# WarranWeng/EBFI-BE

Measured on AMD Instinct MI355X. Metric: interpolated frames/sec (train fwd+bwd) at B=8 256x256, higher is better.
Workload: dtype bf16x3 fwd (f16 KernelConv) / f16 bwd; 1 GPU; EVFIAutoEx (config/train_ours.yml defaults, 5.69 M params) train step: fwd + Lap/census loss + bwd + flat grad all-reduce + Adam; B=8 per GPU, 256x256 frames, TB=16 event bins, Poisson(0.35) event counts; global_batch=8, parallelism=dp1, world_size=1, launch=hipGraph replay of fwd+loss+bwd+grad packing; all-reduce and Adam eager, graph_capture_failed=False, fp16_steps_skipped=0

## Files before the change

ebfi-be_amd/csrc/conv2d.hip:

```cpp
#include <type_traits>

#include "common.hpp"
#include "c16.hpp"

using namespace ebfi;

namespace {

typedef float f32x16 __attribute__((ext_vector_type(16)));

enum { ACT_NONE = 0, ACT_LEAKY = 1, ACT_SIGMOID = 2 };

struct ConvGeom {
    int B, Cin, H, W, Cout, Ho, Wo, pad;
    int groups = 1;
    int store = 0;
};

struct EpiExtra {
    const float *addend;
    const float *mask_y;
    int mask_act;
    float mask_slope;
    _Float16 *out16 = nullptr;
// ... 3781 lines not shown
    }
    {
        ProfScope ps("conv_wgrad_f16_tr/img_batch", st, flops, bytes);
        if (int rc_ = ensure_dynamic_lds(reinterpret_cast<const void *>(&conv_wgrad_f16_tr_batch), TR_LDS + KB_LDS_BYTES)) return rc_;
        hipLaunchKernelGGL(conv_wgrad_f16_tr_batch, dim3((unsigned)(8 * 2 * n * per_xcd)), dim3(512), TR_LDS + KB_LDS_BYTES, st, bt, g0,
                           (int)tiles, per_xcd, n);
        if (int rc = check_launch("conv_wgrad_f16_tr_batch")) return rc;
    }
    {
        ProfScope ps("conv_wgrad_reduce_f32", st);
        hipLaunchKernelGGL(conv_wgrad_reduce_batch, dim3((unsigned)ceil_div(n_total_max, 64), (unsigned)n), dim3(256), 0, st, rb, 8 * per_xcd);
    }
    return check_launch("conv_wgrad_reduce_batch");
}

extern "C" int ebfi_f16_scales_finish(void *slots, int n, void *flag, void *stream) {
    if (!slots || !flag || n < 0) return fail(EBFI_ERR_ARG, "f16_scales_finish: bad argument");
    if (n == 0) return EBFI_OK;
    hipStream_t st = static_cast<hipStream_t>(stream);
    ProfScope ps("f16_scales_finish", st);
    hipLaunchKernelGGL(f16_scales_finish_kernel, dim3((unsigned)ceil_div(n, 256)), dim3(256), 0, st, static_cast<float *>(slots), n,
                       static_cast<int *>(flag));
    return check_launch("f16_scales_finish");
}

extern "C" int ebfi_pack_table_f16(const float *src, const int32_t *table, int64_t n, void *out, const int32_t *block_slot,
                                   void *slots, void *stream) {
    if (!src || !table || !out || !block_slot || !slots) return fail(EBFI_ERR_ARG, "pack_table_f16: null argument");
    if (n <= 0) return EBFI_OK;
    hipStream_t st = static_cast<hipStream_t>(stream);
// ... 39 lines not shown
```

ebfi-be_amd/csrc/conv2d_f16.inc.hpp:

```cpp


constexpr int NTF16 = 512;
template <bool EXTRA, bool IN16 = false, bool INP16 = false, bool FAC = false, bool ST = false>
__global__ __launch_bounds__(NTF16) void conv_fwd_f16_ws(const float *__restrict__ x, const _Float16 *__restrict__ wp,
                                                         const float *__restrict__ bias, float *__restrict__ out, ConvGeom g, int K16,
                                                         int act, float slope, EpiExtra epi, int tiles_total, ScaleSlot in_slot,
                                                         const float *__restrict__ w_slot, FacEpi fac) {
    static_assert(!FAC || (!EXTRA && !INP16), "the FAC epilogue comes without epilogue extras (input: fp32 planes or a c16 image)");
    constexpr int KS = 3, KK = 9, MT = 2, RW = 2;
    constexpr int IH = TYB - 1 + KS, IW = TX - 1 + KS, PS = IH * IW, COS = 32 * MT;
    constexpr int NCW = TYB / RW, PT = 256;
    constexpr int WPIECES = KK * COS * 2, NWB = (WPIECES + PT - 1) / PT;
    constexpr int INB = PS * 32, WB = KK * COS * 32, BUFB = INB + WB;
    static_assert(NCW == 4 && NTF16 == 64 * NCW + PT, "wave roles");
    extern __shared__ __attribute__((aligned(16))) char smd[];
    const int tid = threadIdx.x, lane = tid & 63, wave = tid >> 6;
    const int tiles_x = (g.Wo + TX - 1) / TX, tiles_y = (g.Ho + TYB - 1) / TYB;
    const int co_base = blockIdx.y * COS;
    const int grp = co_base / (g.Cout / g.groups);
    const int HW = g.H * g.W;
    constexpr unsigned ES = INP16 ? 2u : 4u;
    const unsigned plane_bytes = (unsigned)HW * ES, x_bytes = (unsigned)g.Cin * plane_bytes;
    const int nchunks = K16 / CKB;
    const int G = gridDim.x;
// ... 1175 lines not shown
    const int unit = pu % nunits, s_local = pu / nunits;
    WgradItem it = bt.item[0];
#pragma unroll
    for (int k = 1; k < WGRAD_BATCH_MAX; ++k)
        if (unit == k) it = bt.item[k];
    ConvGeom g = g0;
    g.Cin = it.Cin; g.Cout = it.Cout; g.groups = it.groups;
    const int t0 = (int)((int64_t)total_tiles * xcd / 8), t1 = (int)((int64_t)total_tiles * (xcd + 1) / 8);
    const bool two_co = g.Cout > 64;
    const int64_t wsz = (int64_t)g.Cout * g.Cin * 9;
    wgrad_tr_body<ACT_NONE, true, false>(static_cast<const float *>(it.x16), static_cast<const float *>(it.g16), nullptr, nullptr,
                                         it.slab + (int64_t)(xcd * per_xcd + s_local) * (wsz + g.Cout), g, 0.f, t0 + s_local, per_xcd, t1,
                                         false, it.need_bias, ScaleSlot{it.x_slot}, ScaleSlot{it.g_slot}, two_co ? which : 0,
                                         two_co ? 0 : which);
}
```

ebfi-be_amd/csrc/fuse.hip:

```cpp
#include "common.hpp"
#include "c16.hpp"

using namespace ebfi;

namespace {

typedef float f4 __attribute__((ext_vector_type(4)));

__global__ __launch_bounds__(256) void src_fwd_kernel(const float *__restrict__ a0, const float *__restrict__ s0,
                                                      const float *__restrict__ a1, const float *__restrict__ s1,
                                                      const float *__restrict__ x, float *__restrict__ out, int C, int64_t HW4,
                                                      int64_t total4, int64_t a_bs4) {
    const int64_t i = (int64_t)blockIdx.x * 256 + threadIdx.x;
    if (i >= total4) return;
    const int64_t bc = i / HW4, r = i - bc * HW4;
    const int64_t b = bc / C, c = bc - b * C;
    const f4 zero = {0.f, 0.f, 0.f, 0.f};
    const f4 xv = x ? reinterpret_cast<const f4 *>(x)[i] : zero;
    const int64_t ia = b * a_bs4 + c * HW4 + r;
    const f4 v0 = reinterpret_cast<const f4 *>(a0)[ia], v1 = reinterpret_cast<const f4 *>(a1)[ia];
    const float k0 = s0[bc], k1 = s1 ? s1[bc] : 1.f;
    f4 *o = reinterpret_cast<f4 *>(out);
    o[(b * 2 * C + c) * HW4 + r] = v0 * k0 + xv;
    o[(b * 2 * C + C + c) * HW4 + r] = v1 * k1 + xv;
// ... 53 lines not shown
    }
}

__global__ void gather_sum_kernel(const float *__restrict__ src, const int *__restrict__ idx, float *__restrict__ out,
                                  int64_t n_out, int R) {
    const int64_t i = (int64_t)blockIdx.x * blockDim.x + threadIdx.x;
    if (i >= n_out) return;
    float acc = 0.f;
    for (int r = 0; r < R; ++r) {
        const int j = idx[i * R + r];
        if (j >= 0) acc += src[j];
    }
    out[i] = acc;
}

__global__ __launch_bounds__(256) void prodmean_fwd_kernel(const float *__restrict__ a, const float *__restrict__ b,
                                                           float *__restrict__ out, int64_t HW4) {
    __shared__ float red[4];
    const f4 *pa = reinterpret_cast<const f4 *>(a) + (int64_t)blockIdx.x * HW4;
    const f4 *pb = reinterpret_cast<const f4 *>(b) + (int64_t)blockIdx.x * HW4;
    float d = 0.f;
    for (int64_t i = threadIdx.x; i < HW4; i += 256) {
        const f4 u = pa[i], v = pb[i];
        d += (u.x * v.x + u.y * v.y) + (u.z * v.z + u.w * v.w);
    }
#pragma unroll
    for (int s = 32; s >= 1; s >>= 1) d += __shfl_xor(d, s, 64);
    if ((threadIdx.x & 63) == 0) red[threadIdx.x >> 6] = d;
    __syncthreads();
    if (threadIdx.x == 0) out[blockIdx.x] = ((red[0] + red[1]) + (red[2] + red[3])) / (float)(HW4 * 4);
// ... 436 lines not shown
                           static_cast<float *>(slot), grad_x, grad_s0_part, grad_s1_part, B, C, HW / 4, W / 4, (int64_t)0, nslice,
                           mask_slope, static_cast<const float *>(a_slot));
    }
    return check_launch("scale_residual_cat_bwd");
}

extern "C" int ebfi_gather_sum(const float *src, const int32_t *idx, float *out, int64_t n_out, int R, void *stream) {
    if (!src || !idx || !out) return fail(EBFI_ERR_ARG, "gather_sum: null argument");
    if (n_out < 0 || R <= 0) return fail(EBFI_ERR_ARG, "gather_sum: bad dimensions");
    if (n_out == 0) return EBFI_OK;
    hipStream_t st = static_cast<hipStream_t>(stream);
    hipLaunchKernelGGL(gather_sum_kernel, dim3((unsigned)ceil_div(n_out, 256)), dim3(256), 0, st, src, idx, out, n_out, R);
    return check_launch("gather_sum");
}

extern "C" int ebfi_prodmean_forward(const float *a, const float *b, float *out, int64_t planes, int64_t HW, void *stream) {
    if (!a || !b || !out) return fail(EBFI_ERR_ARG, "prodmean_forward: null argument");
    if (planes < 0 || planes > 2147483647LL || HW <= 0) return fail(EBFI_ERR_ARG, "prodmean_forward: bad dimensions");
    if (HW % 4 != 0) return fail(EBFI_ERR_UNSUPPORTED, "prodmean_forward: H*W must be a multiple of 4");
    if (planes == 0) return EBFI_OK;
    hipStream_t st = static_cast<hipStream_t>(stream);
    {
        ProfScope ps("prodmean_fwd", st, 0.0, 8.0 * planes * (double)HW);
        hipLaunchKernelGGL(prodmean_fwd_kernel, dim3((unsigned)planes), dim3(256), 0, st, a, b, out, HW / 4);
    }
    return check_launch("prodmean_fwd");
}

extern "C" int ebfi_prodmean_backward(const float *a, const float *b, const float *grad_out, float *grad_a, float *grad_b,
                                      int64_t planes, int64_t HW, void *stream) {
// ... 57 lines not shown
```

ebfi-be_amd/ebfi_amd/_native.py:

```python
import ctypes
import os
import re
import subprocess
import threading

PKG_ROOT = os.path.dirname(os.path.dirname(os.path.abspath(__file__)))
REPO_ROOT = os.path.dirname(PKG_ROOT)
_DEV = os.environ.get("EBFI_DEV") == "1"


def dev_env(name, default=None):
    return os.environ.get(name, default) if _DEV else default


LIB_PATH = dev_env("EBFI_LIB_PATH") or os.path.join(PKG_ROOT, "lib", "libebfi_hip.so")
HEADER = os.path.join(REPO_ROOT, "include", "ebfi_hip.h")
BUILD_SCRIPT = os.path.join(PKG_ROOT, "csrc", "build.sh")

EBFI_F32, EBFI_F32_BF16MMA, EBFI_F32_BF16X3MMA = 0, 2, 3
EBFI_ERR_UNSUPPORTED = -3
ABI_VERSION = 14


class EbfiNativeError(RuntimeError):
# ... 32 lines not shown
    "ebfi_pack_pairs_block": (_i, []),
    "ebfi_pack_pairs_bf16": (_i, [_vp, _vp, _vp, _vp, _i64, _i64, _vp, _vp]),
    "ebfi_f16_scales_finish": (_i, [_vp, _i, _vp, _vp]),
    "ebfi_pack_table_f16": (_i, [_vp, _vp, _i64, _vp, _vp, _vp, _vp]),
    "ebfi_conv2d_packed_f16": (_i, [_vp, _vp, _sz, _vp, _vp] + [_i] * 8 + [_i, _c.c_float, _vp, _vp, _i, _c.c_float, _vp, _vp, _vp]),
    "ebfi_conv2d_backward_weight_f16g": (_i, [_vp] * 6 + [_i] * 8 + [_i, _c.c_float, _vp, _vp, _vp, _sz, _vp]),
    "ebfi_conv2d_backward_weight_f16g_ex": (_i, [_vp] * 6 + [_i] * 9 + [_i, _c.c_float, _vp, _vp, _vp, _sz, _vp]),
    "ebfi_to_c16": (_i, [_vp, _vp, _c.c_float, _vp, _vp, _i, _i, _i, _i, _vp]),
    "ebfi_to_c16_cat2": (_i, [_vp, _i, _vp, _i, _vp, _vp, _i, _i, _i, _vp]),
    "ebfi_conv2d_packed_x3_c16": (_i, [_vp, _vp, _sz, _vp, _vp] + [_i] * 8 + [_i, _c.c_float, _vp, _vp, _i, _c.c_float, _vp, _vp, _i, _vp]),
    "ebfi_conv2d_packed_f16_c16": (_i, [_vp, _i, _vp, _sz, _vp, _vp] + [_i] * 8 + [_i, _c.c_float, _vp, _vp, _i, _c.c_float,
                                        _vp, _vp, _vp, _vp, _i, _i, _vp]),
    "ebfi_conv2d_backward_weight_f16c": (_i, [_vp, _vp, _i, _vp, _vp] + [_i] * 6 + [_vp, _vp, _vp, _sz, _vp]),
    "ebfi_conv2d_backward_weight_f16c_batch_workspace": (_sz, [_i, _vp, _vp]),
    "ebfi_conv2d_backward_weight_f16c_batch": (_i, [_i] + [_vp] * 9 + [_i, _i, _i, _vp, _sz, _vp]),
    "ebfi_fac_forward_p16": (_i, [_vp, _i, _vp, _vp, _vp, _i, _i, _i, _i, _i, _vp]),
    "ebfi_fac_backward_p16": (_i, [_vp, _i, _vp, _vp, _vp, _vp, _vp, _vp, _c.c_float, _i, _i, _i, _i, _i, _vp]),
    "ebfi_scale_residual_cat_forward_c16": (_i, [_vp] * 8 + [_i, _i, _i, _i, _i64, _vp]),
    "ebfi_scale_residual_cat_backward_slices": (_i, []),
    "ebfi_scale_residual_cat_backward_c16": (_i, [_vp] * 10 + [_i, _i, _i, _i, _i64, _c.c_float, _vp]),
    "ebfi_scale_residual_cat_backward_c16a": (_i, [_vp] * 10 + [_i, _i, _i, _i, _c.c_float, _vp]),
    "ebfi_conv2d_packed_x3_rc": (_i, [_vp, _vp, _sz, _vp, _vp] + [_i] * 6 + [_c.c_float, _vp, _vp, _i, _vp, _vp, _vp, _vp, _vp]),
    "ebfi_conv2d_thin_forward": (_i, [_vp, _vp, _vp, _vp] + [_i] * 8 + [_i, _c.c_float, _vp]),
    "ebfi_kernelconv_fac_fused_x3": (_i, [_vp, _vp, _sz, _vp, _vp, _vp] + [_i] * 6 + [_c.c_float, _vp]),
    "ebfi_kernelconv_fac_fused_f16": (_i, [_vp, _i, _vp, _sz, _vp, _vp, _vp] + [_i] * 6 + [_c.c_float, _vp, _vp, _vp]),
    "ebfi_conv2d_packed_x3": (_i, [_vp, _vp, _sz, _vp, _vp] + [_i] * 8 + [_i, _c.c_float, _vp, _vp, _i, _c.c_float, _vp]),
    "ebfi_conv2d_backward_weight_x3g": (_i, [_vp] * 4 + [_i] * 8 + [_vp, _sz, _vp]),
    "ebfi_scale_residual_cat_forward_ex": (_i, [_vp] * 6 + [_i, _i, _i64, _i64, _vp]),
    "ebfi_scale_residual_cat_backward_ex": (_i, [_vp] * 10 + [_i, _i, _i64, _i64, _i64, _i, _c.c_float, _vp]),
    "ebfi_scalar_conv_forward": (_i, [_vp, _vp, _vp, _vp, _i, _i, _i, _i, _c.c_float, _vp]),
    "ebfi_scalar_conv_backward": (_i, [_vp, _vp, _vp, _vp, _vp, _vp, _vp, _i, _i, _i, _i, _c.c_float, _vp]),
    "ebfi_events_workspace": (_sz, [_i]),
    "ebfi_events_to_stack": (_i, [_vp, _vp, _vp, _vp, _i64, _i, _i, _i, _vp, _vp, _sz, _vp]),
    "ebfi_frame2lap": (_i, [_vp, _vp, _i, _i, _i, _vp]),
    "ebfi_frame2dcp": (_i, [_vp, _vp, _vp, _i, _i, _i, _i, _vp]),
    "ebfi_scale_residual_cat_forward": (_i, [_vp] * 6 + [_i, _i, _i64, _vp]),
    "ebfi_scale_residual_cat_backward": (_i, [_vp] * 10 + [_i, _i, _i64, _vp]),
    "ebfi_prodmean_forward": (_i, [_vp, _vp, _vp, _i64, _i64, _vp]),
    "ebfi_prodmean_backward": (_i, [_vp] * 5 + [_i64, _i64, _vp]),
    "ebfi_gather_sum": (_i, [_vp, _vp, _vp, _i64, _i, _vp]),
    "ebfi_se_gate_workspace": (_c.c_size_t, [_i, _i, _i64]),
    "ebfi_se_gate_forward": (_i, [_vp] * 8 + [_i, _i, _i64, _i, _c.c_float, _vp]),
    "ebfi_se_gate_backward": (_i, [_vp] * 11 + [_i, _i, _i64, _i, _c.c_float, _vp]),
    "ebfi_conv2d_packed_x3_shuffled": (_i, [_vp, _vp, _c.c_size_t, _vp, _vp] + [_i] * 6 + [_c.c_float, _i, _vp]),
    "ebfi_conv2d_packed_f16_shuffled": (_i, [_vp, _i, _vp, _c.c_size_t, _vp, _vp] + [_i] * 6 + [_c.c_float, _vp, _i, _c.c_float, _vp, _vp, _i, _vp]),
    "ebfi_se_gate_forward_ps": (_i, [_vp] * 7 + [_i, _i, _i, _i, _i, _c.c_float, _vp]),
    "ebfi_se_gate_backward_ps": (_i, [_vp] * 10 + [_i, _i, _i, _i, _i, _c.c_float, _vp]),
    "ebfi_groupnorm_workspace": (_sz, [_i, _i]),
    "ebfi_groupnorm_forward": (_i, [_vp] * 6 + [_i, _i, _i64, _i, _c.c_float, _vp, _sz, _vp]),
    "ebfi_groupnorm_backward": (_i, [_vp] * 8 + [_i, _i, _i64, _i, _vp, _sz, _vp]),
    "ebfi_census_partials": (_i64, [_i, _i, _i]),
    "ebfi_census_forward": (_i, [_vp, _vp, _vp, _i, _i, _i, _i, _vp]),
    "ebfi_census_backward": (_i, [_vp, _vp, _vp, _vp, _i, _i, _i, _i, _vp]),
    "ebfi_census_pair_forward": (_i, [_vp, _vp, _vp, _c.c_float, _c.c_float, _vp, _vp, _i, _i, _i, _i, _vp]),
    "ebfi_census_pair_backward": (_i, [_vp, _vp, _vp, _c.c_float, _c.c_float, _vp, _vp, _vp, _i, _i, _i, _i, _vp]),
# ... 177 lines not shown
```

ebfi-be_amd/ebfi_amd/conv.py:

```python
import os

import torch
import torch.nn.functional as F
from torch.autograd import Function

from . import _native as N

ACT_NONE, ACT_LEAKY, ACT_SIGMOID = 0, 1, 2

_COMPUTE = "fp32"
MODES = ("fp32", "bf16x3", "bf16")


def set_compute_dtype(mode):
    global _COMPUTE
    if mode not in MODES:
        raise ValueError("compute dtype must be one of %s" % (MODES,))
    _COMPUTE = mode


def get_compute_dtype():
    return _COMPUTE


# ... 175 lines not shown
        if Cin != site.K:
            raise RuntimeError("input has %d channels, the packed weight expects %d" % (Cin, site.K))
        geo = [B, Cin, H, W, site.M, site.ks, 1, int(pad)]
        Ho, Wo = H + 2 * pad - site.ks + 1, W + 2 * pad - site.ks + 1
        out = torch.empty((B, site.M, Ho, Wo), dtype=x.dtype, device=x.device)
        with torch.cuda.device_of(x):
            if site.kind == "id" and len(site.w_shapes) == 1 and site.groups == 1 and \
                    _thin_forward(x, params[0].contiguous(), site.bias(), out, geo, act, slope):
                rc = 0
            else:
                rc = N.lib().ebfi_conv2d_forward_bf16x3(N.ptr(x), N.ptr(None), N.ptr(site.bias()), N.ptr(out), *geo, act, slope,
                                                        site.fwd_ptr(), site.fwd_bytes, N.stream_ptr(x.device))
        N.check(rc, "ebfi_conv2d_forward_bf16x3 (packed)")
        if grad_preact:
            act, slope = ACT_NONE, 0.0
        ctx.site, ctx.cfg, ctx.geo = site, (act, slope), geo
        ctx.save_for_backward(x, out if act != ACT_NONE else None)
        return out

    @staticmethod
    def backward(ctx, gout):
        x, y = ctx.saved_tensors
        site, (act, slope), geo = ctx.site, ctx.cfg, ctx.geo
        gx, pgrads = _site_backward(site, geo, act, slope, x, y, gout, ctx.needs_input_grad[0], any(ctx.needs_input_grad[6:]))
        return (gx, None, None, None, None, None) + tuple(pgrads)


def _site_backward(site, geo, act, slope, x, y, gout, need_x, need_p, unshuffle=None):
    gout = gout.contiguous()
    lib = N.lib()
    gx, pgrads = None, [None] * (len(site.w_shapes) + len(site.b_shapes))
    from . import f16scale
    book = f16scale.active_book()
    B, Cin, H, W, M, ks, _, pad = geo
    f16 = book is not None and ks == 3 and pad == 1
    al16 = all(t is None or t.data_ptr() % 16 == 0 for t in (x, gout, y))
    f16_w = f16 and (Cin % 64 == 0 or (Cin >= 32 and W % 4 == 0 and al16))
    f16_x = f16 and W % 4 == 0 and Cin >= 48 and site.tr16_ptr() is not None
    gpre = None

    def weight_gradients(st_w):
        gw2 = torch.empty((site.M, site.K, site.ks, site.ks), dtype=x.dtype, device=x.device)
        gb2 = torch.empty(site.M, dtype=x.dtype, device=x.device) if site.has_bias else None
        need = int(lib.ebfi_conv2d_backward_weight_workspace(*geo, N.EBFI_F32))
        ws = torch.empty(max(need, 4), dtype=torch.uint8, device=x.device)
        gpre16 = need_x and act != ACT_NONE and f16_w and f16_x and al16 and W % 4 == 0 and M % 16 == 0 and site.groups == 1
        gp = None
        if need_x and act != ACT_NONE:
            if gpre16:
                from . import c16
                gp = c16.empty(B, M, H, W, x.device)
            else:
                gp = torch.empty_like(gout)
        if f16_w:
            rc = lib.ebfi_conv2d_backward_weight_f16g_ex(N.ptr(x), N.ptr(gout), N.ptr(y), N.ptr(gw2), N.ptr(gb2), N.ptr(gp),
                                                         1 if gpre16 else 0, B, Cin, H, W, M, ks, pad, 1, act, slope,
                                                         book.operand((site.key, "x"), x), book.operand((site.key, "g"), gout),
                                                         N.ptr(ws), need, st_w)
        else:
            rc = lib.ebfi_conv2d_backward_weight_ex(N.ptr(x), N.ptr(gout), N.ptr(y), N.ptr(gw2), N.ptr(gb2), N.ptr(gp), *geo,
                                                    act, slope, N.ptr(ws), need, N.EBFI_F32_BF16X3MMA, st_w)
        N.check(rc, "ebfi_conv2d_backward_weight")
        return _route_site_grads(site, gw2, gb2, st_w), gp

    with torch.cuda.device_of(x):
        st = N.stream_ptr(x.device)
        if need_p:
            pgrads, gpre = weight_gradients(st)
        if need_x:
            src, sy, a = (gpre, None, ACT_NONE) if gpre is not None else (gout, y, act)
            img = gpre is not None and gpre.dtype == torch.float16
            native_unshuffle = unshuffle is not None and (img or (f16_x and a == ACT_NONE)) and site.groups == 1 and H % 2 == 0 and \
                W % 4 == 0 and Cin > 32 and unshuffle[0].is_contiguous() and unshuffle[0].data_ptr() % 16 == 0
            if native_unshuffle:
                gx = torch.empty((B, 4 * Cin, H // 2, W // 2), dtype=x.dtype, device=x.device)
                in_slot = book.ptr(book.slot((site.key, "g"))) if img else book.operand((site.key, "g"), src)
                rc = lib.ebfi_conv2d_packed_f16_shuffled(N.ptr(src), 1 if img else 0, site.tr16_ptr(), site.tr16_bytes, N.ptr(None), N.ptr(gx),
                                                         B, M, H, W, Cin, ACT_NONE, 0.0, N.ptr(unshuffle[0]), ACT_LEAKY, float(unshuffle[1]),
                                                         in_slot, site.w_slot_ptr(), 2, st)
                N.check(rc, "ebfi_conv2d_packed_f16_shuffled (data gradient through the inverse pixel shuffle)")
                return gx, pgrads
            gx = torch.empty_like(x)
# ... 28 lines not shown
        if Cin != site_a.K or site_a.M != 4 * site_b.K:
            raise RuntimeError("shuffled pair: %d -> %d channels, then %d -> %d" % (Cin, site_a.M, site_b.K, site_b.M))
        geo_a = [B, Cin, H, W, site_a.M, 3, 1, 1]
        geo_b = [B, site_b.K, 2 * H, 2 * W, site_b.M, 3, 1, 1]
        y1 = torch.empty((B, site_b.K, 2 * H, 2 * W), dtype=x.dtype, device=x.device)
        y2 = torch.empty((B, site_b.M, 2 * H, 2 * W), dtype=x.dtype, device=x.device)
        with torch.cuda.device_of(x):
            st = N.stream_ptr(x.device)
            rc = N.lib().ebfi_conv2d_packed_x3_shuffled(N.ptr(x), site_a.fwd_ptr(), site_a.fwd_bytes, N.ptr(site_a.bias()), N.ptr(y1), B, Cin,
                                                        H, W, site_a.M, ACT_LEAKY, slope_a, 1, st)
            N.check(rc, "ebfi_conv2d_packed_x3_shuffled")
            rc = N.lib().ebfi_conv2d_forward_bf16x3(N.ptr(y1), N.ptr(None), N.ptr(site_b.bias()), N.ptr(y2), *geo_b, act_b, slope_b,
                                                    site_b.fwd_ptr(), site_b.fwd_bytes, st)
            N.check(rc, "ebfi_conv2d_forward_bf16x3 (packed)")
        ctx.sites, ctx.cfg, ctx.geos, ctx.na = (site_a, site_b), (slope_a, act_b, slope_b), (geo_a, geo_b), na
        ctx.save_for_backward(x, y1, y2 if act_b != ACT_NONE else None)
        return y2

    @staticmethod
    def backward(ctx, g2):
        x, y1, y2 = ctx.saved_tensors
        (site_a, site_b), (slope_a, act_b, slope_b), (geo_a, geo_b), na = ctx.sites, ctx.cfg, ctx.geos, ctx.na
        need = ctx.needs_input_grad
        need_pa, need_pb = any(need[7:7 + na]), any(need[7 + na:])
        need_a = need[0] or need_pa
        ga, pg_b = _site_backward(site_b, geo_b, act_b, slope_b, y1, y2, g2, need_a, need_pb, unshuffle=(y1, slope_a))
        gx, pg_a = (None, [None] * na)
        if need_a:
            gx, pg_a = _site_backward(site_a, geo_a, ACT_NONE, 0.0, x, None, ga, need[0], need_pa)
        return (gx, None, None, None, None, None, None) + tuple(pg_a) + tuple(pg_b)


def shuffle_pair_usable(x, site_a, site_b):
    return (site_usable(site_a, x) and site_b is not None and site_a.ks == 3 and site_b.ks == 3 and site_a.kind == "id" and
            site_b.kind == "id" and site_a.groups == 1 and site_b.groups == 1 and site_a.M == 4 * site_b.K and site_a.M > 32 and
            x.shape[3] % 4 == 0 and x.data_ptr() % 16 == 0 and not torch.is_autocast_enabled())


def conv_shuffle_pair(x, site_a, slope_a, params_a, site_b, act_b, slope_b, params_b):
    return SiteConvShufflePair.apply(x, site_a, float(slope_a), site_b, int(act_b), float(slope_b), len(params_a), *params_a, *params_b)


def _route_site_grads(site, gw2, gb2, st):
    lib = N.lib()
# ... 38 lines not shown
```

ebfi-be_amd/ebfi_amd/engine.py:

```python
import contextlib

import torch

from . import graphstep
from .dp import FlatGradBucket, broadcast_parameters, build_flat_optimizer
from .loss import TrainLoss
from .model import EVFIAutoEx

DEFAULT_MODEL_ARGS = dict(
    FrameBasech=64, EventBasech=64, InterCH=64, TB=16, norm=None, activation="LeakyReLU",
    UseGTEx=False, FixEx=None, BlurryFashion="RGBLap", BLInch=4, UseEvents=True, LoadPretrainEX=False,
    PretrainedEXPath=None, FrozenEX=False, step=12, DualPath=True, residual=True, DetailEnabled=True,
    channels=[16, 24, 32, 64])


def synthetic_batch(B, H, W, TB=16, device="cuda", seed=123, rank=0, on_device=False):
    dev = torch.device(device)
    if on_device and dev.type == "cuda":
        g = torch.Generator(device=dev).manual_seed(seed + rank)
        rnd = lambda *shape: torch.rand(*shape, generator=g, device=dev)
        frame = rnd(B, 3, H, W)
        event = torch.poisson(torch.full((B, TB, 2, H, W), 0.35, device=dev), generator=g)
        t = rnd(B, 1)
        gtex = rnd(B, 1) * 0.4 + 0.55
# ... 27 lines not shown


def synthetic_validation_batch(B, H, W, TB=16, num_frames=4, device="cuda", seed=0):
    g = torch.Generator(device="cpu").manual_seed(int(seed))
    frame = torch.rand(B, 3, H, W, generator=g)
    event = torch.poisson(torch.full((B, TB, 2, H, W), 0.35), generator=g)
    gtex = torch.rand(B, 1, generator=g) * 0.4 + 0.55
    latent = torch.rand(B, num_frames, 3, H, W, generator=g)
    ts = (torch.arange(num_frames) / num_frames).expand(B, num_frames).contiguous()
    return tuple(v.to(device) for v in (frame, event, ts, gtex, latent))


class Engine(graphstep.GraphStepper):
    def __init__(self, model_args=None, device="cuda", precision="fp32", lr=1e-4, seed=None, train=True, graph=False,
                 accu_step=1, betas=(0.9, 0.999), backward_f16=None, forward_f16="filters", strict_graph=None,
                 perceptual=None, optimizer=None):
        if precision not in ("fp32", "bf16x3", "bf16"):
            raise ValueError("precision must be 'fp32', 'bf16x3' or 'bf16'")
        super().__init__(device, graph=graph, accu_step=accu_step, strict_graph=strict_graph)
        self.precision = precision
        if seed is not None:
            torch.manual_seed(seed)
        self.model_args = dict(DEFAULT_MODEL_ARGS, **(model_args or {}))
        self.model = EVFIAutoEx(**self.model_args).to(self.device)
        broadcast_parameters(self.model, 0)
        self.calibration_steps = 2
        self.perceptual = perceptual if train else None
        self.keep_panels, self.panel_sharp, self.last_valid_panels = False, None, None
        if train:
            self.model.train()
            self.loss = TrainLoss(self.model_args.get("DetailEnabled", True)).to(self.device)
            self.bucket = FlatGradBucket(self.model)
            self.optimizer = build_flat_optimizer(self.bucket.params, optimizer, lr, betas)
        else:
            self.model.eval()
        self.bank = None
        if backward_f16 is None:
            backward_f16 = True
        use_book = train and precision == "bf16x3" and backward_f16
        forward_f16 = forward_f16 if use_book else None
        if forward_f16 == "none":
# ... 7 lines not shown
                                             fwd16=forward_f16) if train else weightbank.build_for(self.model, inference=True)
        self.book = None
        if use_book and self.bank is not None:
            from . import f16scale
            self.book = f16scale.ScaleBook(self.device)
            self.bank.attach_scale_book(self.book)
            self.bank.pack_on_demand = True
            self.book.forward_f16 = forward_f16

    def _book(self):
        if self.book is None or self.precision != "bf16x3":
            return contextlib.nullcontext()
        return self.book.active()

    def _fwd_bwd(self, frame, event, t, gtex, target):
        with self._autocast(), self._bank(), self._book() as book:
            if book is not None and self._steps_run < self.calibration_steps:
                book.calibrated.clear()
            sharp_pre, sharp = self.model(frame, event, t, gtex)
            if self.keep_panels:
                if self.panel_sharp is None or self.panel_sharp.shape[1:] != sharp.shape[1:]:
                    self.panel_sharp = torch.empty((1,) + tuple(sharp.shape[1:]), dtype=torch.float32, device=sharp.device)
                self.panel_sharp.copy_(sharp.detach()[:1])
            loss = self.loss(sharp_pre.float(), sharp.float(), target, self.iteration, self.accu_step)
            if self.perceptual is not None:
                loss = loss + self.perceptual(sharp.float(), target) / self.accu_step
            loss.backward()
            if book is not None:
                book.finish()
        return loss.detach()

    def _begin_micro_step(self):
        if self.book is not None and self.precision == "bf16x3" and self._micro == 0:
            self.book.begin_step()

    def _guard(self):
        return self.book.guard if (self.book is not None and self.precision == "bf16x3") else None

    def _calibrating(self):
        return self.book is not None and self.precision == "bf16x3" and self._steps_run < self.calibration_steps

    def _graph_key(self):
# ... 190 lines not shown
```

include/ebfi_hip.h:

```cpp
#ifndef EBFI_HIP_H
#define EBFI_HIP_H

#include <stddef.h>
#include <stdint.h>

#ifdef __cplusplus
extern "C" {
#endif

#define EBFI_ABI_VERSION 14

typedef enum {
    EBFI_OK = 0,
    EBFI_ERR_ARG = -1,
    EBFI_ERR_LAUNCH = -2,
    EBFI_ERR_UNSUPPORTED = -3,
    EBFI_ERR_WORKSPACE = -4
} ebfi_status;

typedef enum { EBFI_F32 = 0, EBFI_F32_BF16MMA = 2, EBFI_F32_BF16X3MMA = 3 } ebfi_dtype;

int ebfi_abi_version(void);
const char *ebfi_last_error(void);

// ... 132 lines not shown
int ebfi_conv2d_packed_x3_shuffled(const void *input, const void *packed, size_t packed_bytes, const void *bias, void *output,
                                   int B, int Cin, int H, int W, int Cout, int act, float slope, int out_layout, void *stream);
int ebfi_conv2d_packed_f16_shuffled(const void *input, int input_is_c16, const void *packed16, size_t packed_bytes,
                                    const void *bias, void *output, int B, int Cin, int H, int W, int Cout, int act, float slope,
                                    const void *mask_y, int mask_act, float mask_slope, void *in_slot, const void *w_slot,
                                    int out_layout, void *stream);
int ebfi_conv2d_backward_weight_f16c(const void *input16, const void *grad16, int grad_is_planar, void *grad_weight,
                                     void *grad_bias, int B, int Cin_per_group, int H, int W, int Cout, int groups,
                                     const void *x_slot, const void *g_slot, void *workspace, size_t workspace_bytes,
                                     void *stream);
size_t ebfi_conv2d_backward_weight_f16c_batch_workspace(int n, const int *Cin_per_group, const int *Cout);
int ebfi_conv2d_backward_weight_f16c_batch(int n, const void *const *input16, const void *const *grad16, void *const *grad_weight,
                                           void *const *grad_bias, const int *Cin_per_group, const int *Cout, const int *groups,
                                           void *const *x_slot, void *const *g_slot, int B, int H, int W, void *workspace,
                                           size_t workspace_bytes, void *stream);
int ebfi_fac_forward_p16(const float *input, int input_is_unpadded, const void *filters16, const void *f_slot, float *output, int B,
                         int C, int Ho, int Wo, int K, void *stream);
int ebfi_fac_backward_p16(const float *input, int input_is_unpadded, const void *filters16, const void *f_slot,
                          const float *grad_output, float *grad_input, void *grad_kernel16, void *g_slot, float kernel_leaky_slope,
                          int B, int C, int Ho, int Wo, int K, void *stream);
int ebfi_scale_residual_cat_forward_c16(const float *a0, const float *s0, const float *a1, const float *s1, const float *x,
                                        float *out, void *out16, void *slot, int B, int C, int H, int W,
                                        int64_t a_batch_stride, void *stream);
int ebfi_scale_residual_cat_backward_slices(void);
int ebfi_scale_residual_cat_backward_c16(const float *grad_out, const float *a0, const float *s0, const float *a1,
                                         const float *s1, void *grad_a16, void *slot, float *grad_x, float *grad_s0_part,
                                         float *grad_s1_part, int B, int C, int H, int W, int64_t a_batch_stride,
                                         float mask_slope, void *stream);
int ebfi_scale_residual_cat_backward_c16a(const float *grad_out, const void *a16, const void *a_slot, const float *s0, const float *s1,
                                          void *grad_a16, void *slot, float *grad_x, float *grad_s0_part, float *grad_s1_part, int B,
// ... 27 lines not shown
                                     const float *s1, float *grad_a0, float *grad_a1, float *grad_x,
                                     float *grad_s0, float *grad_s1, int B, int C, int64_t HW, void *stream);

int ebfi_scale_residual_cat_forward_ex(const float *a0, const float *s0, const float *a1, const float *s1, const float *x,
                                       float *out, int B, int C, int64_t HW, int64_t a_batch_stride, void *stream);
int ebfi_scale_residual_cat_backward_ex(const float *grad_out, const float *a0, const float *s0, const float *a1,
                                        const float *s1, float *grad_a0, float *grad_a1, float *grad_x, float *grad_s0,
                                        float *grad_s1, int B, int C, int64_t HW, int64_t a_batch_stride,
                                        int64_t grad_a_batch_stride, int mask_leaky, float mask_slope, void *stream);

int ebfi_prodmean_forward(const float *a, const float *b, float *out, int64_t planes, int64_t HW, void *stream);
int ebfi_prodmean_backward(const float *a, const float *b, const float *grad_out, float *grad_a, float *grad_b,
                           int64_t planes, int64_t HW, void *stream);

int ebfi_gather_sum(const float *src, const int32_t *idx, float *out, int64_t n_out, int R, void *stream);

size_t ebfi_se_gate_workspace(int B, int C, int64_t N);
int ebfi_se_gate_forward(const float *x, const float *weight, const float *bias, const float *res, float *out, float *mean,
                         float *gate, float *workspace, int B, int C, int64_t N, int act, float slope, void *stream);
int ebfi_se_gate_backward(const float *grad_out, const float *out, const float *x, const float *weight, const float *gate,
                          const float *mean, float *grad_x, float *grad_res, float *grad_weight, float *grad_bias,
                          float *workspace, int B, int C, int64_t N, int act, float slope, void *stream);

int ebfi_se_gate_forward_ps(const float *x, const float *weight, const float *bias, float *out, float *mean, float *gate,
                            float *workspace, int B, int C, int h, int w, int act, float slope, void *stream);
int ebfi_se_gate_backward_ps(const float *grad_out, const float *out, const float *x, const float *weight, const float *gate,
                             const float *mean, float *grad_x, float *grad_weight, float *grad_bias, float *workspace, int B, int C,
                             int h, int w, int act, float slope, void *stream);

size_t ebfi_groupnorm_workspace(int B, int C);
// ... 148 lines not shown
```

Before: 568.7 frames/s.

## Defer conv weight gradients into a batched multi-layer wgrad and gather launch

Adds a weight-gradient queue that collects eligible 3x3 conv layers during backward and computes all their weight gradients at the end in one grouped kernel plus one grouped reduce. Per-parameter gather-sum routing is batched the same way through a multi-item gather kernel. The aim is fewer small launches and better GPU fill for small layers whose wgrad underuses the device. In exchange, activations and output gradients stay alive until the flush, which raises peak memory, and wgrad work no longer overlaps with the dgrad chain.

```diff
diff --git a/ebfi-be_amd/csrc/conv2d.hip b/ebfi-be_amd/csrc/conv2d.hip
--- a/ebfi-be_amd/csrc/conv2d.hip
+++ b/ebfi-be_amd/csrc/conv2d.hip
@@ -3819,6 +3819,121 @@
     return check_launch("conv_wgrad_reduce_batch");
 }
 
+namespace {
+struct ReduceMultiItem {
+    const float *slab;
+    float *gw, *gb;
+    int64_t n_weight, n_total;
+    int perm_cin, nslabs;
+};
+struct ReduceMulti {
+    ReduceMultiItem item[WGRAD_MULTI_MAX];
+};
+__global__ __launch_bounds__(256) void conv_wgrad_reduce_multi(ReduceMulti rb) {
+    const ReduceMultiItem &it = rb.item[blockIdx.y];
+    if ((int64_t)blockIdx.x * 64 >= it.n_total) return;
+    wgrad_reduce_body(it.slab, it.nslabs, it.n_weight, it.n_total, it.gw, it.gb, it.perm_cin, 9);
+}
+
+int64_t wgrad_multi_tiles(const ConvGeom &g) { return (int64_t)g.B * ceil_div(g.Ho, TRH) * ceil_div(g.Wo, TRW); }
+void wgrad_multi_plan(const ConvGeom *g, int n, int *nsplit) {
+    for (int k = 0; k < n; ++k) {
+        const int64_t tiles = wgrad_multi_tiles(g[k]);
+        const int s = wgrad_x3_splits(g[k], 3);
+        nsplit[k] = (int)(s > tiles ? tiles : s);
+    }
+}
+size_t wgrad_multi_slab_bytes(const ConvGeom &g, int nsplit) {
+    const size_t b = (size_t)nsplit * ((size_t)g.Cout * g.Cin * 9 + g.Cout) * sizeof(float);
+    return (b + 255) / 256 * 256;
+}
+}
+
+extern "C" size_t ebfi_conv2d_backward_weight_f16g_multi_workspace(int n, const int *B, const int *Cin, const int *H, const int *W,
+                                                                   const int *Cout) {
+    if (n < 1 || !B || !Cin || !H || !W || !Cout) return 0;
+    size_t total = 0;
+    for (int k0 = 0; k0 < n; k0 += WGRAD_MULTI_MAX) {
+        const int m = n - k0 < WGRAD_MULTI_MAX ? n - k0 : WGRAD_MULTI_MAX;
+        ConvGeom g[WGRAD_MULTI_MAX];
+        int ns[WGRAD_MULTI_MAX];
+        for (int k = 0; k < m; ++k)
+            if (B[k0 + k] < 1 || make_geom(g[k], B[k0 + k], Cin[k0 + k], H[k0 + k], W[k0 + k], Cout[k0 + k], 3, 1, 1) != EBFI_OK) return 0;
+        wgrad_multi_plan(g, m, ns);
+        for (int k = 0; k < m; ++k) total += wgrad_multi_slab_bytes(g[k], ns[k]);
+    }
+    return total;
+}
+
+extern "C" int ebfi_conv2d_backward_weight_f16g_multi(int n, const void *const *input, const void *const *grad_output,
+                                                      void *const *grad_weight, void *const *grad_bias, const int *B, const int *Cin,
+                                                      const int *H, const int *W, const int *Cout, const int *ksize, const int *stride,
+                                                      const int *pad, const int *groups, void *const *x_slot, void *const *g_slot,
+                                                      void *workspace, size_t workspace_bytes, void *stream) {
+    if (n < 1) return fail(EBFI_ERR_ARG, "conv2d_backward_weight_f16g_multi: %d layers", n);
+    if (!input || !grad_output || !grad_weight || !grad_bias || !B || !Cin || !H || !W || !Cout || !ksize || !stride || !pad || !groups ||
+        !x_slot || !g_slot)
+        return fail(EBFI_ERR_ARG, "conv2d_backward_weight_f16g_multi: null argument");
+    for (int k = 0; k < n; ++k) {
+        if (!input[k] || !grad_output[k] || !grad_weight[k]) return fail(EBFI_ERR_ARG, "conv2d_backward_weight_f16g_multi: null argument (layer %d)", k);
+        if (ksize[k] != 3 || stride[k] != 1 || pad[k] != 1 || groups[k] != 1 || B[k] < 1 || Cin[k] < 16 || W[k] % 4 != 0 ||
+            !aligned16(input[k]) || !aligned16(grad_output[k]))
+            return fail(EBFI_ERR_UNSUPPORTED, "conv2d_backward_weight_f16g_multi: layer %d (k=%d stride %d pad %d, %d groups, %d -> %d channels, "
+                                              "W=%d) is not a 3x3 same-padded stride-1 layer on quad-aligned rows with >= 16 input channels and "
+                                              "16-byte aligned operands", k, ksize[k], stride[k], pad[k], groups[k], Cin[k], Cout[k], W[k]);
+        ConvGeom g;
+        if (int rc = make_geom(g, B[k], Cin[k], H[k], W[k], Cout[k], 3, 1, 1)) return rc;
+        if (shift_wgrad_geometry(g, 3, 1).kind != 0 || thin_wgrad_geometry(g, 3, 1).kind != 0)
+            return fail(EBFI_ERR_UNSUPPORTED, "conv2d_backward_weight_f16g_multi: layer %d (%d -> %d) is a thin layer with kernels of its own", k,
+                        Cin[k], Cout[k]);
+        if (wgrad_multi_tiles(g) > 2147483647LL / 4) return fail(EBFI_ERR_ARG, "conv2d_backward_weight_f16g_multi: too many tiles (layer %d)", k);
+    }
+    const size_t need = ebfi_conv2d_backward_weight_f16g_multi_workspace(n, B, Cin, H, W, Cout);
+    if (!workspace || workspace_bytes < need)
+        return fail(EBFI_ERR_WORKSPACE, "conv2d_backward_weight_f16g_multi: workspace %zu bytes < required %zu", workspace_bytes, need);
+    hipStream_t st = static_cast<hipStream_t>(stream);
+    char *ws = static_cast<char *>(workspace);
+    for (int k0 = 0; k0 < n; k0 += WGRAD_MULTI_MAX) {
+        const int m = n - k0 < WGRAD_MULTI_MAX ? n - k0 : WGRAD_MULTI_MAX;
+        ConvGeom g[WGRAD_MULTI_MAX];
+        int ns[WGRAD_MULTI_MAX];
+        for (int k = 0; k < m; ++k) (void)make_geom(g[k], B[k0 + k], Cin[k0 + k], H[k0 + k], W[k0 + k], Cout[k0 + k], 3, 1, 1);
+        wgrad_multi_plan(g, m, ns);
+        WgradMulti mt{};
+        ReduceMulti rb{};
+        double flops = 0.0, bytes = 0.0;
+        int64_t wgs = 0, n_total_max = 0;
+        for (int k = 0; k < m; ++k) {
+            const int i = k0 + k;
+            const int64_t n_weight = (int64_t)g[k].Cout * g[k].Cin * 9, n_total = n_weight + g[k].Cout;
+            float *slab = reinterpret_cast<float *>(ws);
+            ws += wgrad_multi_slab_bytes(g[k], ns[k]);
+            mt.item[k] = WgradMultiItem{static_cast<const float *>(input[i]), static_cast<const float *>(grad_output[i]), slab,
+                                        static_cast<float *>(x_slot[i]), static_cast<float *>(g_slot[i]), g[k].B, g[k].Cin, g[k].H, g[k].W,
+                                        g[k].Cout, ns[k], (int)wgrad_multi_tiles(g[k]), grad_bias[i] != nullptr ? 1 : 0, (int)wgs, 0};
+            rb.item[k] = ReduceMultiItem{slab, static_cast<float *>(grad_weight[i]), static_cast<float *>(grad_bias[i]), n_weight, n_total,
+                                         g[k].Cin, ns[k]};
+            wgs += ceil_div((int64_t)ns[k] * ceil_div(g[k].Cout, 64) * ceil_div(g[k].Cin, 64), 8) * 8;
+            n_total_max = n_total > n_total_max ? n_total : n_total_max;
+            flops += 2.0 * g[k].B * g[k].Ho * g[k].Wo * (double)g[k].Cout * g[k].Cin * 9;
+            bytes += conv_bytes_wgrad(g[k], 9, false, false);
+        }
+        if (wgs > 2147483647LL) return fail(EBFI_ERR_ARG, "conv2d_backward_weight_f16g_multi: too many workgroups");
+        {
+            ProfScope ps("conv_wgrad_f16_tr/f32_multi", st, flops, bytes);
+            if (int rc_ = ensure_dynamic_lds(reinterpret_cast<const void *>(&conv_wgrad_f16_tr_multi), TR_LDS + KB_LDS_BYTES)) return rc_;
+            hipLaunchKernelGGL(conv_wgrad_f16_tr_multi, dim3((unsigned)wgs), dim3(512), TR_LDS + KB_LDS_BYTES, st, mt, m);
+            if (int rc = check_launch("conv_wgrad_f16_tr_multi")) return rc;
+        }
+        {
+            ProfScope ps("conv_wgrad_reduce_f32", st);
+            hipLaunchKernelGGL(conv_wgrad_reduce_multi, dim3((unsigned)ceil_div(n_total_max, 64), (unsigned)m), dim3(256), 0, st, rb);
+            if (int rc = check_launch("conv_wgrad_reduce_multi")) return rc;
+        }
+    }
+    return EBFI_OK;
+}
+
 extern "C" int ebfi_f16_scales_finish(void *slots, int n, void *flag, void *stream) {
     if (!slots || !flag || n < 0) return fail(EBFI_ERR_ARG, "f16_scales_finish: bad argument");
     if (n == 0) return EBFI_OK;
diff --git a/ebfi-be_amd/csrc/conv2d_f16.inc.hpp b/ebfi-be_amd/csrc/conv2d_f16.inc.hpp
--- a/ebfi-be_amd/csrc/conv2d_f16.inc.hpp
+++ b/ebfi-be_amd/csrc/conv2d_f16.inc.hpp
@@ -1213,3 +1213,44 @@
                                          false, it.need_bias, ScaleSlot{it.x_slot}, ScaleSlot{it.g_slot}, two_co ? which : 0,
                                          two_co ? 0 : which);
 }
+
+struct WgradMultiItem {
+    const float *x, *gout;
+    float *slab, *x_slot, *g_slot;
+    int B, Cin, H, W, Cout;
+    int nsplit, total_tiles, need_bias;
+    int wg_begin, pad_;
+};
+constexpr int WGRAD_MULTI_MAX = 16;
+struct WgradMulti {
+    WgradMultiItem item[WGRAD_MULTI_MAX];
+};
+__global__ __launch_bounds__(512) void conv_wgrad_f16_tr_multi(WgradMulti mt, int n) {
+    int k = 0;
+    for (int j = 1; j < n; ++j)
+        if ((int)blockIdx.x >= mt.item[j].wg_begin) k = j;
+    const WgradMultiItem &it = mt.item[k];
+    const int nx = it.nsplit, ny = (it.Cout + 63) / 64, nz = (it.Cin + 63) / 64;
+    const int L = (int)blockIdx.x - it.wg_begin, total = nx * ny * nz;
+    if (L >= total) return;
+    int split, co_blk, ci_blk;
+    {
+        const int T8 = total / (8 * nz) * (8 * nz);
+        int rest;
+        if (L < T8) {
+            const int xcd = L & 7, i = L >> 3;
+            ci_blk = i % nz;
+            rest = (i / nz) * 8 + xcd;
+        } else {
+            ci_blk = (L - T8) % nz;
+            rest = T8 / nz + (L - T8) / nz;
+        }
+        split = rest % nx;
+        co_blk = rest / nx;
+    }
+    ConvGeom g{it.B, it.Cin, it.H, it.W, it.Cout, it.H, it.W, 1};
+    const int64_t wsz = (int64_t)g.Cout * g.Cin * 9;
+    wgrad_tr_body<ACT_NONE, false, false>(it.x, it.gout, nullptr, nullptr, it.slab + (int64_t)split * (wsz + g.Cout), g, 0.f, split, nx,
+                                          it.total_tiles, (nx & 7) == 0, it.need_bias, ScaleSlot{it.x_slot}, ScaleSlot{it.g_slot},
+                                          co_blk, ci_blk, 0);
+}
diff --git a/ebfi-be_amd/csrc/fuse.hip b/ebfi-be_amd/csrc/fuse.hip
--- a/ebfi-be_amd/csrc/fuse.hip
+++ b/ebfi-be_amd/csrc/fuse.hip
@@ -91,6 +91,35 @@
     out[i] = acc;
 }
 
+struct GatherItem {
+    const float *src;
+    const int *idx;
+    float *out;
+    int64_t n_out;
+    int R, wg_begin;
+};
+constexpr int GATHER_MULTI_MAX = 48;
+struct GatherMulti {
+    GatherItem item[GATHER_MULTI_MAX];
+};
+__global__ __launch_bounds__(256) void gather_sum_multi_kernel(GatherMulti gm, int n) {
+    int k = 0;
+    for (int j = 1; j < n; ++j)
+        if ((int)blockIdx.x >= gm.item[j].wg_begin) k = j;
+    const GatherItem &it = gm.item[k];
+    const int64_t i = (int64_t)((int)blockIdx.x - it.wg_begin) * 256 + threadIdx.x;
+    if (i >= it.n_out) return;
+    const int R = it.R;
+    const int *__restrict__ idx = it.idx;
+    const float *__restrict__ src = it.src;
+    float acc = 0.f;
+    for (int r = 0; r < R; ++r) {
+        const int j = idx[i * R + r];
+        if (j >= 0) acc += src[j];
+    }
+    it.out[i] = acc;
+}
+
 __global__ __launch_bounds__(256) void prodmean_fwd_kernel(const float *__restrict__ a, const float *__restrict__ b,
                                                            float *__restrict__ out, int64_t HW4) {
     __shared__ float red[4];
@@ -557,6 +586,37 @@
     return check_launch("gather_sum");
 }
 
+extern "C" int ebfi_gather_sum_multi(int n, const float *const *src, const int32_t *const *idx, float *const *out, const int64_t *n_out,
+                                     const int *R, void *stream) {
+    if (n < 0 || !src || !idx || !out || !n_out || !R) return fail(EBFI_ERR_ARG, "gather_sum_multi: bad argument");
+    for (int k = 0; k < n; ++k) {
+        if (!src[k] || !idx[k] || !out[k]) return fail(EBFI_ERR_ARG, "gather_sum_multi: null argument (item %d)", k);
+        if (n_out[k] < 0 || R[k] <= 0) return fail(EBFI_ERR_ARG, "gather_sum_multi: bad dimensions (item %d)", k);
+    }
+    hipStream_t st = static_cast<hipStream_t>(stream);
+    int k = 0;
+    while (k < n) {
+        GatherMulti gm{};
+        int m = 0;
+        int64_t wgs = 0;
+        for (; k < n && m < GATHER_MULTI_MAX; ++k) {
+            if (n_out[k] == 0) continue;
+            const int64_t w = ceil_div(n_out[k], 256);
+            if (wgs + w > 2147483647LL) {
+                if (m == 0) return fail(EBFI_ERR_ARG, "gather_sum_multi: item %d is too large", k);
+                break;
+            }
+            gm.item[m++] = GatherItem{src[k], idx[k], out[k], n_out[k], R[k], (int)wgs};
+            wgs += w;
+        }
+        if (m == 0) break;
+        ProfScope ps("gather_sum", st);
+        hipLaunchKernelGGL(gather_sum_multi_kernel, dim3((unsigned)wgs), dim3(256), 0, st, gm, m);
+        if (int rc = check_launch("gather_sum_multi")) return rc;
+    }
+    return EBFI_OK;
+}
+
 extern "C" int ebfi_prodmean_forward(const float *a, const float *b, float *out, int64_t planes, int64_t HW, void *stream) {
     if (!a || !b || !out) return fail(EBFI_ERR_ARG, "prodmean_forward: null argument");
     if (planes < 0 || planes > 2147483647LL || HW <= 0) return fail(EBFI_ERR_ARG, "prodmean_forward: bad dimensions");
diff --git a/ebfi-be_amd/ebfi_amd/_native.py b/ebfi-be_amd/ebfi_amd/_native.py
--- a/ebfi-be_amd/ebfi_amd/_native.py
+++ b/ebfi-be_amd/ebfi_amd/_native.py
@@ -70,6 +70,8 @@
     "ebfi_conv2d_backward_weight_f16c": (_i, [_vp, _vp, _i, _vp, _vp] + [_i] * 6 + [_vp, _vp, _vp, _sz, _vp]),
     "ebfi_conv2d_backward_weight_f16c_batch_workspace": (_sz, [_i, _vp, _vp]),
     "ebfi_conv2d_backward_weight_f16c_batch": (_i, [_i] + [_vp] * 9 + [_i, _i, _i, _vp, _sz, _vp]),
+    "ebfi_conv2d_backward_weight_f16g_multi_workspace": (_sz, [_i] + [_vp] * 5),
+    "ebfi_conv2d_backward_weight_f16g_multi": (_i, [_i] + [_vp] * 15 + [_vp, _sz, _vp]),
     "ebfi_fac_forward_p16": (_i, [_vp, _i, _vp, _vp, _vp, _i, _i, _i, _i, _i, _vp]),
     "ebfi_fac_backward_p16": (_i, [_vp, _i, _vp, _vp, _vp, _vp, _vp, _vp, _c.c_float, _i, _i, _i, _i, _i, _vp]),
     "ebfi_scale_residual_cat_forward_c16": (_i, [_vp] * 8 + [_i, _i, _i, _i, _i64, _vp]),
@@ -95,6 +97,7 @@
     "ebfi_prodmean_forward": (_i, [_vp, _vp, _vp, _i64, _i64, _vp]),
     "ebfi_prodmean_backward": (_i, [_vp] * 5 + [_i64, _i64, _vp]),
     "ebfi_gather_sum": (_i, [_vp, _vp, _vp, _i64, _i, _vp]),
+    "ebfi_gather_sum_multi": (_i, [_i, _vp, _vp, _vp, _vp, _vp, _vp]),
     "ebfi_se_gate_workspace": (_c.c_size_t, [_i, _i, _i64]),
     "ebfi_se_gate_forward": (_i, [_vp] * 8 + [_i, _i, _i64, _i, _c.c_float, _vp]),
     "ebfi_se_gate_backward": (_i, [_vp] * 11 + [_i, _i, _i64, _i, _c.c_float, _vp]),
diff --git a/ebfi-be_amd/ebfi_amd/conv.py b/ebfi-be_amd/ebfi_amd/conv.py
--- a/ebfi-be_amd/ebfi_amd/conv.py
+++ b/ebfi-be_amd/ebfi_amd/conv.py
@@ -213,7 +213,7 @@
         N.check(rc, "ebfi_conv2d_forward_bf16x3 (packed)")
         if grad_preact:
             act, slope = ACT_NONE, 0.0
-        ctx.site, ctx.cfg, ctx.geo = site, (act, slope), geo
+        ctx.site, ctx.cfg, ctx.geo, ctx.params = site, (act, slope), geo, params
         ctx.save_for_backward(x, out if act != ACT_NONE else None)
         return out
 
@@ -221,11 +221,12 @@
     def backward(ctx, gout):
         x, y = ctx.saved_tensors
         site, (act, slope), geo = ctx.site, ctx.cfg, ctx.geo
-        gx, pgrads = _site_backward(site, geo, act, slope, x, y, gout, ctx.needs_input_grad[0], any(ctx.needs_input_grad[6:]))
+        gx, pgrads = _site_backward(site, geo, act, slope, x, y, gout, ctx.needs_input_grad[0], any(ctx.needs_input_grad[6:]),
+                                    params=(ctx.params, ctx.needs_input_grad[6:]))
         return (gx, None, None, None, None, None) + tuple(pgrads)
 
 
-def _site_backward(site, geo, act, slope, x, y, gout, need_x, need_p, unshuffle=None):
+def _site_backward(site, geo, act, slope, x, y, gout, need_x, need_p, unshuffle=None, params=None):
     gout = gout.contiguous()
     lib = N.lib()
     gx, pgrads = None, [None] * (len(site.w_shapes) + len(site.b_shapes))
@@ -237,6 +238,8 @@
     f16_w = f16 and (Cin % 64 == 0 or (Cin >= 32 and W % 4 == 0 and al16))
     f16_x = f16 and W % 4 == 0 and Cin >= 48 and site.tr16_ptr() is not None
     gpre = None
+    from . import wgradqueue
+    queue = wgradqueue.active() if params is not None and need_p and wgradqueue.deferrable(*params) else None
 
     def weight_gradients(st_w):
         gw2 = torch.empty((site.M, site.K, site.ks, site.ks), dtype=x.dtype, device=x.device)
@@ -260,11 +263,16 @@
             rc = lib.ebfi_conv2d_backward_weight_ex(N.ptr(x), N.ptr(gout), N.ptr(y), N.ptr(gw2), N.ptr(gb2), N.ptr(gp), *geo,
                                                     act, slope, N.ptr(ws), need, N.EBFI_F32_BF16X3MMA, st_w)
         N.check(rc, "ebfi_conv2d_backward_weight")
+        if queue is not None and site.kind != "id":
+            queue.add_routes(site, gw2, gb2, *params)
+            return pgrads, gp
         return _route_site_grads(site, gw2, gb2, st_w), gp
 
     with torch.cuda.device_of(x):
         st = N.stream_ptr(x.device)
-        if need_p:
+        if need_p and queue is not None and f16_w and wgradqueue.eligible(site, geo, act, x, gout):
+            queue.add_layer(site, x, gout, geo, book.operand((site.key, "x"), x), book.operand((site.key, "g"), gout), *params)
+        elif need_p:
             pgrads, gpre = weight_gradients(st)
         if need_x:
             src, sy, a = (gpre, None, ACT_NONE) if gpre is not None else (gout, y, act)
@@ -323,6 +331,7 @@
                                                     site_b.fwd_ptr(), site_b.fwd_bytes, st)
             N.check(rc, "ebfi_conv2d_forward_bf16x3 (packed)")
         ctx.sites, ctx.cfg, ctx.geos, ctx.na = (site_a, site_b), (slope_a, act_b, slope_b), (geo_a, geo_b), na
+        ctx.params = params
         ctx.save_for_backward(x, y1, y2 if act_b != ACT_NONE else None)
         return y2
 
@@ -333,10 +342,12 @@
         need = ctx.needs_input_grad
         need_pa, need_pb = any(need[7:7 + na]), any(need[7 + na:])
         need_a = need[0] or need_pa
-        ga, pg_b = _site_backward(site_b, geo_b, act_b, slope_b, y1, y2, g2, need_a, need_pb, unshuffle=(y1, slope_a))
+        ga, pg_b = _site_backward(site_b, geo_b, act_b, slope_b, y1, y2, g2, need_a, need_pb, unshuffle=(y1, slope_a),
+                                  params=(ctx.params[na:], need[7 + na:]))
         gx, pg_a = (None, [None] * na)
         if need_a:
-            gx, pg_a = _site_backward(site_a, geo_a, ACT_NONE, 0.0, x, None, ga, need[0], need_pa)
+            gx, pg_a = _site_backward(site_a, geo_a, ACT_NONE, 0.0, x, None, ga, need[0], need_pa,
+                                      params=(ctx.params[:na], need[7:7 + na]))
         return (gx, None, None, None, None, None, None) + tuple(pg_a) + tuple(pg_b)
 
 
diff --git a/ebfi-be_amd/ebfi_amd/engine.py b/ebfi-be_amd/ebfi_amd/engine.py
--- a/ebfi-be_amd/ebfi_amd/engine.py
+++ b/ebfi-be_amd/ebfi_amd/engine.py
@@ -65,7 +65,7 @@
 class Engine(graphstep.GraphStepper):
     def __init__(self, model_args=None, device="cuda", precision="fp32", lr=1e-4, seed=None, train=True, graph=False,
                  accu_step=1, betas=(0.9, 0.999), backward_f16=None, forward_f16="filters", strict_graph=None,
-                 perceptual=None, optimizer=None):
+                 perceptual=None, optimizer=None, defer_wgrad=True, defer_wgrad_cap=None):
         if precision not in ("fp32", "bf16x3", "bf16"):
             raise ValueError("precision must be 'fp32', 'bf16x3' or 'bf16'")
         super().__init__(device, graph=graph, accu_step=accu_step, strict_graph=strict_graph)
@@ -76,6 +76,7 @@
         self.model = EVFIAutoEx(**self.model_args).to(self.device)
         broadcast_parameters(self.model, 0)
         self.calibration_steps = 2
+        self.defer_wgrad, self.defer_wgrad_cap = bool(defer_wgrad), defer_wgrad_cap
         self.perceptual = perceptual if train else None
         self.keep_panels, self.panel_sharp, self.last_valid_panels = False, None, None
         if train:
@@ -113,7 +114,10 @@
         return self.book.active()
 
     def _fwd_bwd(self, frame, event, t, gtex, target):
-        with self._autocast(), self._bank(), self._book() as book:
+        from . import wgradqueue
+        cap = wgradqueue.BYTE_CAP if self.defer_wgrad_cap is None else self.defer_wgrad_cap
+        with self._autocast(), self._bank(), self._book() as book, \
+                wgradqueue.scope(self.defer_wgrad and self.book is not None, cap) as queue:
             if book is not None and self._steps_run < self.calibration_steps:
                 book.calibrated.clear()
             sharp_pre, sharp = self.model(frame, event, t, gtex)
@@ -125,6 +129,8 @@
             if self.perceptual is not None:
                 loss = loss + self.perceptual(sharp.float(), target) / self.accu_step
             loss.backward()
+            if queue is not None:
+                queue.flush()
             if book is not None:
                 book.finish()
         return loss.detach()
diff --git a/ebfi-be_amd/ebfi_amd/wgradqueue.py b/ebfi-be_amd/ebfi_amd/wgradqueue.py
--- /dev/null
+++ b/ebfi-be_amd/ebfi_amd/wgradqueue.py
@@ -0,0 +1,140 @@
+import contextlib
+import ctypes
+
+import torch
+
+from . import _native as N
+
+BYTE_CAP = 1 << 30
+
+_ACTIVE = None
+
+
+def active():
+    return _ACTIVE
+
+
+def deferrable(params, needs):
+    return all((not n) or (p.is_leaf and p.requires_grad) for p, n in zip(params, needs))
+
+
+def eligible(site, geo, act, x, gout):
+    B, Cin, H, W, M, ks, _, pad = geo
+    return (act == 0 and ks == 3 and pad == 1 and site.groups == 1 and W % 4 == 0 and Cin >= 16 and B >= 1 and
+            x.data_ptr() % 16 == 0 and gout.data_ptr() % 16 == 0 and
+            not (B * H * W >= 65536 and (M <= 4 or Cin <= 4)))
+
+
+def _vps(vals):
+    return (ctypes.c_void_p * len(vals))(*vals)
+
+
+def _ints(vals):
+    return (ctypes.c_int * len(vals))(*[int(v) for v in vals])
+
+
+class WgradQueue:
+    def __init__(self, byte_cap=BYTE_CAP):
+        self.byte_cap = int(byte_cap)
+        self.layers = []
+        self.gathers = []
+        self.bytes = 0
+        self.flushes = 0
+
+    def add_layer(self, site, x, gout, geo, x_slot, g_slot, params, needs):
+        self.layers.append((site, x, gout, list(geo), x_slot, g_slot, list(params), list(needs)))
+        self._held(x.numel() * x.element_size() + gout.numel() * gout.element_size())
+
+    def add_routes(self, site, gw2, gb2, params, needs, count=True):
+        nw = len(site.w_shapes)
+        if site.kind == "id":
+            row = 0
+            for p, need, shp in zip(params[:nw], needs[:nw], site.w_shapes):
+                if need:
+                    _assign(p, gw2[row:row + shp[0]].view(shp))
+                row += shp[0]
+            row = 0
+            for p, need, shp in zip(params[nw:], needs[nw:], site.b_shapes):
+                if need:
+                    _assign(p, gb2[row:row + shp[0]].view(shp))
+                row += shp[0]
+            return
+        for p, need, shp, inv, R in zip(params[:nw], needs[:nw], site.w_shapes, site.w_inv, site.w_R):
+            if need:
+                self.gathers.append((gw2, inv, int(R), shp, p))
+        for p, need, shp, inv, R in zip(params[nw:], needs[nw:], site.b_shapes, site.b_inv, site.b_R):
+            if need:
+                self.gathers.append((gb2, inv, int(R), shp, p))
+        if count:
+            self._held(gw2.numel() * 4)
+
+    def _held(self, nbytes):
+        self.bytes += int(nbytes)
+        if self.bytes > self.byte_cap:
+            self.flush()
+
+    def flush(self):
+        layers, self.layers = self.layers, []
+        if layers:
+            self._run_layers(layers)
+        gathers, self.gathers = self.gathers, []
+        if gathers:
+            self._run_gathers(gathers)
+        self.bytes = 0
+        self.flushes += 1
+
+    def _run_layers(self, layers):
+        lib = N.lib()
+        dev = layers[0][1].device
+        n = len(layers)
+        gws, gbs = [], []
+        for site, x, gout, geo, xs, gs, params, needs in layers:
+            gws.append(torch.empty((site.M, site.K, 3, 3), dtype=x.dtype, device=dev))
+            gbs.append(torch.empty(site.M, dtype=x.dtype, device=dev) if site.has_bias else None)
+        col = lambda i: _ints([L[3][i] for L in layers])
+        Bs, Cins, Hs, Ws, Couts = col(0), col(1), col(2), col(3), col(4)
+        need = int(lib.ebfi_conv2d_backward_weight_f16g_multi_workspace(n, Bs, Cins, Hs, Ws, Couts))
+        if need == 0:
+            raise N.EbfiNativeError("ebfi_conv2d_backward_weight_f16g_multi_workspace refused the queued layers")
+        ws = torch.empty(need, dtype=torch.uint8, device=dev)
+        slot = lambda v: v.value if isinstance(v, ctypes.c_void_p) else v
+        with torch.cuda.device(dev):
+            rc = lib.ebfi_conv2d_backward_weight_f16g_multi(
+                n, _vps([L[1].data_ptr() for L in layers]), _vps([L[2].data_ptr() for L in layers]),
+                _vps([g.data_ptr() for g in gws]), _vps([None if g is None else g.data_ptr() for g in gbs]),
+                Bs, Cins, Hs, Ws, Couts, col(5), col(6), col(7), _ints([L[0].groups for L in layers]),
+                _vps([slot(L[4]) for L in layers]), _vps([slot(L[5]) for L in layers]), N.ptr(ws), need, N.stream_ptr(dev))
+        N.check(rc, "ebfi_conv2d_backward_weight_f16g_multi")
+        for (site, x, gout, geo, xs, gs, params, needs), gw2, gb2 in zip(layers, gws, gbs):
+            self.add_routes(site, gw2, gb2, params, needs, count=False)
+
+    def _run_gathers(self, gathers):
+        lib = N.lib()
+        dev = gathers[0][0].device
+        outs = [torch.empty(shp, dtype=src.dtype, device=dev) for src, inv, R, shp, p in gathers]
+        n = len(gathers)
+        with torch.cuda.device(dev):
+            rc = lib.ebfi_gather_sum_multi(n, _vps([g[0].data_ptr() for g in gathers]), _vps([g[1].data_ptr() for g in gathers]),
+                                           _vps([o.data_ptr() for o in outs]), (ctypes.c_int64 * n)(*[o.numel() for o in outs]),
+                                           _ints([g[2] for g in gathers]), N.stream_ptr(dev))
+        N.check(rc, "ebfi_gather_sum_multi")
+        for (src, inv, R, shp, p), out in zip(gathers, outs):
+            _assign(p, out)
+
+
+def _assign(p, g):
+    p.grad = g if p.grad is None else p.grad + g
+
+
+@contextlib.contextmanager
+def scope(enabled=True, byte_cap=BYTE_CAP):
+    global _ACTIVE
+    if not enabled:
+        yield None
+        return
+    prev, _ACTIVE = _ACTIVE, WgradQueue(byte_cap)
+    try:
+        yield _ACTIVE
+    finally:
+        q, _ACTIVE = _ACTIVE, prev
+        q.layers, q.gathers = [], []
diff --git a/include/ebfi_hip.h b/include/ebfi_hip.h
--- a/include/ebfi_hip.h
+++ b/include/ebfi_hip.h
@@ -170,6 +170,12 @@
                                            void *const *grad_bias, const int *Cin_per_group, const int *Cout, const int *groups,
                                            void *const *x_slot, void *const *g_slot, int B, int H, int W, void *workspace,
                                            size_t workspace_bytes, void *stream);
+size_t ebfi_conv2d_backward_weight_f16g_multi_workspace(int n, const int *B, const int *Cin, const int *H, const int *W, const int *Cout);
+int ebfi_conv2d_backward_weight_f16g_multi(int n, const void *const *input, const void *const *grad_output, void *const *grad_weight,
+                                           void *const *grad_bias, const int *B, const int *Cin, const int *H, const int *W,
+                                           const int *Cout, const int *ksize, const int *stride, const int *pad, const int *groups,
+                                           void *const *x_slot, void *const *g_slot, void *workspace, size_t workspace_bytes,
+                                           void *stream);
 int ebfi_fac_forward_p16(const float *input, int input_is_unpadded, const void *filters16, const void *f_slot, float *output, int B,
                          int C, int Ho, int Wo, int K, void *stream);
 int ebfi_fac_backward_p16(const float *input, int input_is_unpadded, const void *filters16, const void *f_slot,
@@ -227,6 +233,8 @@
                            int64_t planes, int64_t HW, void *stream);
 
 int ebfi_gather_sum(const float *src, const int32_t *idx, float *out, int64_t n_out, int R, void *stream);
+int ebfi_gather_sum_multi(int n, const float *const *src, const int32_t *const *idx, float *const *out, const int64_t *n_out,
+                          const int *R, void *stream);
 
 size_t ebfi_se_gate_workspace(int B, int C, int64_t N);
 int ebfi_se_gate_forward(const float *x, const float *weight, const float *bias, const float *res, float *out, float *mean,
```

After: 580.3 frames/s (median of 6 runs). 1.02x the previous value.
